# entn-at/tf-kaldi-speaker

Hardware: AMD Instinct MI355X
Metric: utterances/sec x-vector extraction (30-dim x 300-frame) (higher is better)
Workload: dtype f16+fp6-cross(f32-split); 1 GPU; tdnn x-vector (tdnn6_dense), statistics_pooling, 256 utt/GPU/step of 300 frames x 30 dims; batch_per_gpu=256, frames=300, node=tdnn6_dense, precision=f16f6, parallelism=utterance-shard x1, launch=stream launches

## Files before the change

### __graft_entry__.py

```python
import os
import subprocess
import sys

ROOT = os.path.dirname(os.path.abspath(__file__))
PKG = os.path.join(ROOT, "tf-kaldi-speaker_amd")
CSRC = os.path.join(PKG, "csrc")
LIB = os.path.join(PKG, "libxvec_hip.so")
SOURCES = ["gemm_f32.hip", "gemm_bf16x3.hip", "gemm_f6v2.hip", "gemm_f16f6.hip", "pool.hip", "grid.hip", "frontend.hip", "post.hip", "score.hip", "xvec_api.hip", "ark_io.cpp"]


AUDITED = ("gemm_bf16x3.hip", "gemm_f6v2.hip")


def audit_resources(remarks):
    import re
    kernels, cur = {}, None
    for line in remarks.splitlines():
        m = re.search(r"remark: Function Name: (\S+)", line)
        if m:
            cur = kernels.setdefault(m.group(1), {})
            continue
        m = re.search(r"remark:\s+([A-Za-z ]+?)(?: \[[^\]]*\])?: (\S+) \[-Rpass", line)
        if m and cur is not None:
            cur[m.group(1).strip()] = m.group(2)
    rows, bad = [], []
    for name, r in sorted(kernels.items()):
        if "w14p2" not in name and "w1p3" not in name and "gemm_f6v2_kernel" not in name:
            continue
        need_occ = 3
        rows.append("%s VGPRs %s SGPRs %s scratch %s vgpr_spill %s sgpr_spill %s occupancy %s"
                    % (name, r.get("VGPRs"), r.get("TotalSGPRs"), r.get("ScratchSize"), r.get("VGPRs Spill"),
                       r.get("SGPRs Spill"), r.get("Occupancy")))
        if r.get("ScratchSize") != "0" or r.get("VGPRs Spill") != "0" or int(r.get("Occupancy", "0")) < need_occ:
            bad.append(rows[-1])
    if len(rows) < 4:
        raise RuntimeError("resource audit: expected the hand-scheduled w14p2 / w1p3 kernels in the compiler remarks, found %d" % len(rows))
    os.makedirs(os.path.join(ROOT, "profiles", "r03"), exist_ok=True)
    with open(os.path.join(ROOT, "profiles", "r03", "gemm_resources.txt"), "w") as f:
        f.write("# hipcc -Rpass-analysis=kernel-resource-usage, csrc/gemm_bf16x3.hip + csrc/gemm_f6v2.hip (written by __graft_entry__.build)\n")
        f.write("\n".join(rows) + "\n")
    if bad:
        raise RuntimeError("resource audit failed (scratch / VGPR spill / too low an occupancy in a hand-counted-vmcnt kernel):\n"
                           + "\n".join(bad))
    print("[build] resource audit ok: %d hand-scheduled kernels, no scratch, no VGPR spill" % len(rows))


def audit_asm(asm_jobs):
    sys.path.insert(0, os.path.join(ROOT, "tools"))
    import asm_guard
    rows, bad = [], []
    for proc, cmd, asm in asm_jobs:
        if proc.wait() != 0:
            raise subprocess.CalledProcessError(proc.returncode, cmd)
        r, b = asm_guard.check_file(asm, want=("w14p2", "w1p3", "gemm_f6v2_kernel"), local=("w14p2", "w1p3"))
        rows += r
        bad += b
    if len(rows) < 4:
        raise RuntimeError("asm guard: expected the hand-scheduled kernels in the assembly, found %d" % len(rows))
    with open(os.path.join(ROOT, "profiles", "r03", "asm_guard.txt"), "w") as f:
        f.write("# tools/asm_guard.py on hipcc -S --cuda-device-only of csrc/gemm_bf16x3.hip + csrc/gemm_f6v2.hip (written by __graft_entry__.build)\n")
        f.write("\n".join(rows) + "\n")
    if bad:
        raise RuntimeError("asm guard failed:\n" + "\n".join(bad[:20]))
    print("[build] asm guard ok: %d kernels, no in-flight register touched, no compiler vector-memory instruction in a K loop" % len(rows))


def _stale():
    if not os.path.isfile(LIB):
        return True
    t = os.path.getmtime(LIB)
    deps = [os.path.join(CSRC, f) for f in os.listdir(CSRC)] + [os.path.join(ROOT, "include", "xvec_hip.h")]
    return any(os.path.getmtime(d) > t for d in deps)


def build(force=False):
    if force or _stale():
        objdir = os.path.join(PKG, "build")
        os.makedirs(objdir, exist_ok=True)
        flags = ["-O3", "-std=c++17", "--offload-arch=gfx950", "-fPIC", "-I", os.path.join(ROOT, "include")]
        flags += os.environ.get("XVEC_EXTRA_CFLAGS", "").split()
        jobs, asm_jobs = [], []
        for src in SOURCES:
            obj = os.path.join(objdir, os.path.splitext(src)[0] + ".o")
            cmd = ["hipcc"] + flags + ["-c", os.path.join(CSRC, src), "-o", obj]
            audit = src in AUDITED
            if audit:
                cmd.insert(1, "-Rpass-analysis=kernel-resource-usage")
# ... 61 lines not shown
```

### tf-kaldi-speaker_amd/csrc/gemm_bf16x3.hip

```cpp
#include <cstdlib>
#include <mutex>

#include "xv_f6.h"

namespace xv {

namespace {
constexpr int BM = 128, BN = 128;
constexpr int ROWB = 144;
constexpr int TILE_B = BM * ROWB;
typedef int i32x4 __attribute__((ext_vector_type(4)));
}

namespace {
constexpr int DROW = 128;
constexpr int DA_ROWS = 136;
constexpr int DA_BYTES = DA_ROWS * DROW;
constexpr int DB_BYTES = BN * DROW;
typedef __attribute__((address_space(1))) const void* gptr_t;
typedef __attribute__((address_space(3))) void* lptr_t;
}

#ifdef XV_LAB
__global__ __launch_bounds__(256, 2) void gemm_bf16x3_kernel(GemmArgs p, int nMt, int nNt) {
// ... 610 lines not shown
    mt = nMt + tile / nNt;
    nt = tile % nNt;
    const int per = cb_end / S;
    cb_begin = split * per;
    cb_end = cb_begin + per;
    p.Y = p.partial + ((int64_t)split * p.tail_mt - nMt) * (int64_t)BM * p.Npad;
    p.ldy = p.Npad;
    slice = true;
  } else if (EPI == 0 && (int)blockIdx.x >= nMt * nNt) {
    const int id = blockIdx.x - nMt * nNt;
    const int split = id % S, tile = id / S;
    mt = nMt + tile / nNt;
    nt = tile % nNt;
    const int per = cb_end / S;
    cb_begin = split * per;
    cb_end = cb_begin + per;
    p.Y = p.partial + ((int64_t)split * p.tail_mt - nMt) * (int64_t)BM * p.Npad;
    p.raw = 1;
    p.act = ACT_NONE;
    p.alpha = nullptr;
    p.ldy = p.Npad;
    p.N = p.Npad;
    p.M = (nMt + p.tail_mt) * BM;
    p.Ysb = nullptr;
    p.rowmap = nullptr;
    p.R = nullptr;
    p.pool_part = nullptr;
  } else {
    tile_of_block(blockIdx.x, nMt, nNt, mt, nt);
  }
  w14p2_tile<NPS, EPI, F16>(p, mt * BM, nt * BN, w, smem3, cb_begin, cb_end, slice);
}

__global__ void bf16x3_tail_reduce_kernel(GemmArgs p, int mt0, int S) {
  const int quads = p.Npad >> 2;
  const int64_t rows = (int64_t)p.tail_mt * BM;
  const int64_t total = rows * quads;
  for (int64_t i = (int64_t)blockIdx.x * blockDim.x + threadIdx.x; i < total; i += (int64_t)gridDim.x * blockDim.x) {
    const int64_t r = i / quads;
    const int n = (int)(i - r * quads) * 4;
    const int64_t m = (int64_t)mt0 * BM + r;
    if (m >= p.M) continue;
    bool zero;
    const int orow = out_row(p, (int)m, zero);
    if (orow < 0) continue;
    f32x4 acc = {0.f, 0.f, 0.f, 0.f};
    for (int s = 0; s < S; ++s) acc += *reinterpret_cast<const f32x4*>(p.partial + ((int64_t)s * rows + r) * p.Npad + n);
    f32x4 v = {0.f, 0.f, 0.f, 0.f};
#pragma unroll
    for (int e = 0; e < 4; ++e)
      if (n + e < p.N && !zero) v[e] = apply_act(fmaf(acc[e], p.scale[n + e], p.shift[n + e]), p.act, p.alpha ? p.alpha[n + e] : 0.f);
    if (p.Y && n < p.N) *reinterpret_cast<f32x4*>(p.Y + (int64_t)orow * p.ldy + n) = v;
    if (p.Ysb && n < p.ldsb) {
      uint32_t h01, l01, h23, l23;
      v *= p.sb_mul;
      split2(v[0], v[1], h01, l01, p.f16);
      split2(v[2], v[3], h23, l23, p.f16);
      if (p.f16) ovf_report(p.ovf, fmaxf(fmaxf(fabsf(v[0]), fabsf(v[1])), fmaxf(fabsf(v[2]), fabsf(v[3]))));
      char* blk = reinterpret_cast<char*>(p.Ysb) + (int64_t)orow * p.ldsb * 4 + (n >> 5) * 128 + (n & 31) * 2;
      *reinterpret_cast<uint2*>(blk) = make_uint2(h01, h23);
      *reinterpret_cast<uint2*>(blk + 64) = make_uint2(l01, l23);
    }
  }
}

#undef XV_GLD
// ... 154 lines not shown
    else       hipLaunchKernelGGL((gemm_bf16x3_w1p3_kernel<0, false, true>), grid, block, smemw1p3, s, a, nMain, nNt);
    return hipGetLastError();
  }
  if (a.ysb_f6 && (!a.f16 || (w > 1 && w < 5) || !a.Ysb || a.Y || a.R || a.pool_part)) return hipErrorInvalidValue;
  if (w == 1 && !tail && a.slab3) {
    if (a.ysb_f6) hipLaunchKernelGGL((gemm_bf16x3_w1p3_kernel<3, true>), grid, block, smemw1p3, s, a, nMain, nNt);
    else if (a.f16) hipLaunchKernelGGL((gemm_bf16x3_w1p3_kernel<0, true>), grid, block, smemw1p3, s, a, nMain, nNt);
    else       hipLaunchKernelGGL((gemm_bf16x3_w1p3_kernel<0, false>), grid, block, smemw1p3, s, a, nMain, nNt);
    return hipGetLastError();
  }
  const int S = tail ? a.ksplit : 0;
  const dim3 grid2(nMain * nNt + (tail ? a.tail_mt * nNt * a.ksplit : 0));
  if (a.ysb_f6) {
    if (w >= 5) hipLaunchKernelGGL((gemm_bf16x3_w14p2_kernel<1, 3, true>), grid2, block, smemw32, s, a, nMain, nNt, w, S);
    else        hipLaunchKernelGGL((gemm_bf16x3_w14p2_kernel<4, 3, true>), grid2, block, smemw32, s, a, nMain, nNt, w, S);
    const hipError_t e6 = hipGetLastError();
    if (e6 != hipSuccess || !tail) return e6;
    return launch_f6v2_tail_reduce(a, nMain, s);
  }
  if (w >= 5) {
    if (a.f16) hipLaunchKernelGGL((gemm_bf16x3_w14p2_kernel<1, 0, true>), grid2, block, smemw32, s, a, nMain, nNt, w, S);
    else       hipLaunchKernelGGL((gemm_bf16x3_w14p2_kernel<1, 0, false>), grid2, block, smemw32, s, a, nMain, nNt, w, S);
  } else {
    if (a.f16) hipLaunchKernelGGL((gemm_bf16x3_w14p2_kernel<4, 0, true>), grid2, block, smemw32, s, a, nMain, nNt, w, S);
    else       hipLaunchKernelGGL((gemm_bf16x3_w14p2_kernel<4, 0, false>), grid2, block, smemw32, s, a, nMain, nNt, w, S);
  }
  hipError_t e = hipGetLastError();
  if (e != hipSuccess || !tail) return e;
  const int64_t total = (int64_t)a.tail_mt * BM * (a.Npad >> 2);
  hipLaunchKernelGGL(bf16x3_tail_reduce_kernel, dim3((unsigned)((total + 255) / 256)), block, 0, s, a, nMain, a.ksplit);
  return hipGetLastError();
}

}

#ifdef XV_GEMM_TRACE
extern "C" int xvdbg_gemm_trace(long long* out, int max_wgs) {
  if (!xv::g_trace || xv::g_trace_wgs <= 0) return 0;
  const int n = xv::g_trace_wgs < max_wgs ? xv::g_trace_wgs : max_wgs;
  if (hipDeviceSynchronize() != hipSuccess) return -1;
  if (hipMemcpy(out, xv::g_trace, sizeof(long long) * 8 * n, hipMemcpyDeviceToHost) != hipSuccess) return -1;
  return n;
}
#endif
```

### tf-kaldi-speaker_amd/csrc/xv_kernels.h

```cpp
#pragma once
#include <hip/hip_runtime.h>
#include <stdint.h>

namespace xv {

enum Act : int { ACT_NONE = 0, ACT_RELU = 1, ACT_LRELU = 2, ACT_PRELU = 3, ACT_TANH = 4 };

constexpr float kLreluAlpha = 0.2f;
constexpr int kFlagWords = 8, kUttSmallWord = 4, kFeatMaxSlots = 32768;
constexpr float kVarFloor = 1e-12f;

struct GemmArgs {
  const float* X;
  int64_t ldx;
  int cin;
  int M;
  int K;
  int N;
  const float* Wt;
  int Kpad;
  int Npad;
  const float* scale;
  const float* shift;
  const float* alpha;
// ... 22 lines not shown
  int tail_mt = 0;
  float* pool_part;
  const int32_t* pool_row2utt;
  const int32_t* pool_slotbase;
  int64_t a_pitch;
  int64_t a_off;
  int64_t tap_stride;
  int ntaps;
  int ktap;
  const int32_t* arow;
  const float* R;
  int64_t ldr;
  const float* att_q = nullptr;
  float* att_part = nullptr;
  int64_t att_ld = 0;
  int att_heads = 0;
  const float* pool_w = nullptr;
  int pool_heads = 0;
  int pool_split = 0;
  int pool_dvh = 0;
  int pool_odim = 0;
};

hipError_t launch_gemm_f32(const GemmArgs& a, bool aligned, hipStream_t s);

int gemm_f32_ksplit(int M, int Kpad, int Npad);

int64_t gemm_bf16x3_tail_plan(int M, int Kpad, int Npad, int w, int* tail_mt, int* splits, int cb_quant = 1);

hipError_t launch_im2col_sb(const float* x, int64_t ldx, int cin, int w, int64_t rows, void* out_sb, int ldsb, int f16,
                            int* ovf, hipStream_t s);

hipError_t launch_gemm_bf16x3(const GemmArgs& a, hipStream_t s);
hipError_t launch_gemm_f16f6(const GemmArgs& a, hipStream_t s);
hipError_t launch_f6v2_tail_reduce(const GemmArgs& a, int nMain, hipStream_t s);
hipError_t launch_f6_from_sb(const void* sb, void* out, int64_t rows, int nblk, hipStream_t s);

hipError_t launch_build_rowmap(const int32_t* off0, int B, int ctx_in, int w, int32_t* rowmap, int M,
                               hipStream_t s);

hipError_t launch_stat_pool(const float* x, int64_t ldx, int C, const int32_t* off0, int B, int ctx,
                            float* out, int64_t ldo, hipStream_t s);

hipError_t launch_build_row2utt(const int32_t* off0, int B, int ctx, int32_t* row2utt, int M, hipStream_t s);
hipError_t launch_pool_finalize(const float* part, int C, const int32_t* off0, int B, int ctx,
                                const int32_t* slotbase, float* out, int64_t ldo, hipStream_t s);

hipError_t launch_build_rowmap_grid(const int32_t* off0, int B, int rows_per_t, int Fout, int So, int cover, int32_t* rowmap,
                                    int64_t M, hipStream_t s);
hipError_t launch_build_rowmap_grid_ts(const int32_t* off_in, const int32_t* off_out, int B, int rows_per_t, int Fout, int So,
                                       int ktime, int32_t* rowmap, int64_t M, hipStream_t s);
hipError_t launch_build_rowmap_grid_compact(const int32_t* off_in, const int32_t* off_out, int B, int Sin, int So, int Fout,
                                            int sw, int st, int ktime, int32_t* arow, int32_t* rowmap, int64_t M, int64_t Mpad,
                                            hipStream_t s);
hipError_t launch_grid_zero_border(const int32_t* off0, int B, int64_t frames, int F, int S, int chunks_y, int chunks_sb,
                                   float* y, void* ysb, hipStream_t s);
hipError_t launch_build_rowmap_rows(const int32_t* off0, int B, int32_t* rowmap, int64_t M, hipStream_t s);
hipError_t launch_build_rowmap_trows(const int32_t* off0, int B, int So, int32_t* rowmap, int64_t M, hipStream_t s);
hipError_t launch_build_rowmap_interior(const int32_t* off0, int B, int F, int S, int32_t* rowmap, int64_t M, hipStream_t s);
hipError_t launch_im2col2d_sb(const float* x, int64_t ldx, const int32_t* off0, int B, int F, int S, int64_t P, void* out_sb,
                              int f16, int* ovf, hipStream_t s);
hipError_t launch_im2col2d_f32(const float* x, int64_t ldx, const int32_t* off0, int B, int F, int S, int64_t P, float* out,
                               hipStream_t s);
hipError_t launch_conv0_direct(const float* x, int64_t ldx, const int32_t* off0, int B, int F, int S, int C, int64_t P,
                               const float* wdir, int act, const float* alpha, float* y, void* ysb, int ldsb, int f16, int* ovf,
                               float sb_mul, hipStream_t s);
// ... 67 lines not shown
```

### tf-kaldi-speaker_amd/csrc/xvec_api.hip

```cpp
#include <hip/hip_runtime.h>

#include <algorithm>
#include <cmath>
#include <cstdarg>
#include <cstdio>
#include <cstring>
#include <map>
#include <mutex>
#include <string>
#include <vector>

#include "../../include/xvec_hip.h"
#include "xv_kernels.h"

using namespace xv;

namespace {

constexpr double kBnEps = 1e-3;
constexpr int kSlackRows = 512;
constexpr int kAlign = 256;

thread_local std::string g_last_error;

// ... 86 lines not shown
  int sb_exp = 0;
};

struct Op {
  int kind = OP_GEMM;
  int layer = -1;
  int in0 = -1, in1 = -1;
  int out = -1;
  int bnvec = -1;
};

struct Node {
  std::string name;
  int op = -1;
  int stage = -1;
  bool att_weights = false;
};

}

struct xv_handle {
  xv_model_desc desc{};
  int device = 0;
  bool finalized = false;
  std::string err;
  std::mutex mu;
  std::mutex err_mu;
  std::mutex prof_mu;
  int opt_pool_fusion = 1;
  int opt_tail_split = 1;
  int opt_onetap_f6_notail = 1;
  int opt_grid_f6 = 1;
  int opt_slab3 = 1;
  int opt_grid_compact = 1;
  int opt_att_fusion = 1;
  int opt_profile_dominant = 0;
  std::mutex pool_mu;
  std::vector<DevBuf> pool;
  size_t pool_bytes = 0;
  std::map<std::string, HostTensor> tensors;
  std::vector<Layer> layers;
  std::vector<Value> values;
  std::vector<Op> ops;
  std::vector<Node> nodes;
  DevBuf query;
  DevBuf ovf_flag;
  DevBuf query_eff;
  int key_npad = 0;
  int att_dk_h = 0, att_dk = 0, att_dv = 0;
  int final_ctx = 14;
  std::string post_bn_scope, post_alpha_name;
  DevBuf post_vec;
  int pool_dim = 0;
  struct ProfRec { hipEvent_t e0, e1; const xv_plan* plan; int step; };
  bool profiling = false;
  std::vector<hipEvent_t> prof_pool;
  size_t prof_next = 0;
  std::vector<ProfRec> prof_recs;
  int prof_forwards = 0;
};

struct PlanStep {
  int op = -1;
  int stage = -1;
  bool to_out = false;
  int64_t out_off = -1;
  int64_t out_sb_off = -1;
  int64_t in0_off = -1, in1_off = -1;
  int64_t in0_sb_off = -1;
  int64_t rows_in = 0, rows_out = 0;
  int M = 0;
  int rowmap = -1;
  int64_t scratch_off = -1;
  int64_t scratch2_off = -1;
  int ksplit = 1;
  int tail_mt = 0;
  bool fuse_pool = false;
  int lvl_in = 0, lvl_out = 0;
  int64_t frames_out = 0;
  bool grid_cover = false;
  bool out_f6 = false;
  bool trows = false;
  bool in_f6 = false;
  bool compact = false;
  int arow = -1;
  int fuse_att = 0;
  int64_t att_w_off = -1;
  int64_t att_s0_off = -1;
  int64_t att_ld = 0;
  bool unpad_to_out = false;
  int64_t flops = 0, bytes = 0;
};

struct xv_plan {
  xv_handle* h = nullptr;
  xv_plan_info info{};
  std::vector<int32_t> offsets;
  std::vector<int32_t> offsets_slotbase;
  DevBuf d_offsets;
  std::vector<int32_t> lvl_offsets[4];
  DevBuf d_lvl[4];
  const int32_t* dev_offsets(int level) const {
    return static_cast<const int32_t*>(level > 0 ? d_lvl[level].p : d_offsets.p);
  }
  DevBuf d_rowmaps;
  std::vector<int64_t> rowmap_off;
  std::vector<PlanStep> steps;
  DevBuf d_row2utt;
  DevBuf d_slotbase;
  int64_t pool_slots = 0;
  bool uniform_len = true;
  int uniform_L = 0;
  int dominant_step = 0;
};

namespace {

int fail(xv_handle* h, int code, const char* fmt, ...) {
  char buf[512];
  va_list ap;
  va_start(ap, fmt);
  vsnprintf(buf, sizeof(buf), fmt, ap);
  va_end(ap);
  if (h) {
    std::lock_guard<std::mutex> lk(h->err_mu);
    h->err = buf;
  }
  g_last_error = buf;
  return code;
}

#define XV_HIP(h, expr)                                                                              \
  do {                                                                                               \
    hipError_t _e = (expr);                                                                          \
    if (_e != hipSuccess)                                                                            \
      return fail((h), XV_ERR_HIP, "%s failed: %s (%s:%d)", #expr, hipGetErrorString(_e), __FILE__,  \
                  __LINE__);                                                                         \
  } while (0)

int64_t align_up(int64_t v, int64_t a) { return (v + a - 1) / a * a; }

constexpr size_t kPoolMaxBuffers = 96, kPoolMaxBytes = (size_t)1 << 30;
// ... 732 lines not shown
        }
      XV_HIP(h, h->query_eff.alloc(qe.size() * sizeof(float)));
      XV_HIP(h, hipMemcpy(h->query_eff.p, qe.data(), qe.size() * sizeof(float), hipMemcpyHostToDevice));
    }
    if (h->desc.att_apply_nonlinear) {
      const int n = h->pool_dim;
      std::vector<double> s, t;
      bn_fold(h, h->post_bn_scope, n, s, t);
      std::vector<float> vec((size_t)3 * n, 0.f);
      for (int i = 0; i < n; ++i) { vec[i] = (float)s[i]; vec[(size_t)n + i] = (float)t[i]; }
      if (!h->post_alpha_name.empty()) {
        const auto& a = T(h, h->post_alpha_name).data;
        for (int i = 0; i < n; ++i) vec[(size_t)2 * n + i] = a[i];
      }
      XV_HIP(h, h->post_vec.alloc(vec.size() * sizeof(float)));
      XV_HIP(h, hipMemcpy(h->post_vec.p, vec.data(), vec.size() * sizeof(float), hipMemcpyHostToDevice));
    }
  }
  XV_HIP(h, h->ovf_flag.alloc((kFlagWords + kFeatMaxSlots) * sizeof(int)));
  XV_HIP(h, hipMemset(h->ovf_flag.p, 0, (kFlagWords + kFeatMaxSlots) * sizeof(int)));
  XV_HIP(h, hipDeviceSynchronize());
  for (auto& kv : h->tensors) { kv.second.data.clear(); kv.second.data.shrink_to_fit(); }
  h->finalized = true;
  return XV_OK;
}

int xv_set_option(xv_handle* h, const char* name, int value) {
  if (!h || !name) return fail(h, XV_ERR_INVALID, "xv_set_option: null argument");
  std::lock_guard<std::mutex> lk(h->mu);
  if (!strcmp(name, "pool_fusion")) h->opt_pool_fusion = value != 0;
  else if (!strcmp(name, "tail_split")) h->opt_tail_split = value != 0;
  else if (!strcmp(name, "att_fusion")) h->opt_att_fusion = value != 0;
  else if (!strcmp(name, "slab3")) h->opt_slab3 = value != 0;
  else if (!strcmp(name, "onetap_f6_notail")) h->opt_onetap_f6_notail = value != 0;
  else if (!strcmp(name, "grid_f6")) h->opt_grid_f6 = value != 0;
  else if (!strcmp(name, "grid_compact")) h->opt_grid_compact = value != 0;
  else if (!strcmp(name, "profile_dominant")) h->opt_profile_dominant = value != 0;
  else return fail(h, XV_ERR_INVALID, "xv_set_option: unknown option '%s'", name);
  return XV_OK;
}

int xv_check_overflow(xv_handle* h, int reset) {
  if (!h) return fail(nullptr, XV_ERR_INVALID, "xv_check_overflow: null handle");
  if (!h->finalized || !h->ovf_flag.p) return 0;
  DeviceGuard g(h->device);
  std::vector<int32_t> w((size_t)kFlagWords + kFeatMaxSlots);
  XV_HIP(h, hipMemcpy(w.data(), h->ovf_flag.p, w.size() * sizeof(int32_t), hipMemcpyDeviceToHost));
  int32_t v[2] = {w[0], w[1]};
  for (int i = 0; i < kFeatMaxSlots; ++i) v[1] = std::max(v[1], w[(size_t)kFlagWords + i]);
  if (w[kUttSmallWord]) v[1] = w[kUttSmallWord];
  if (reset) XV_HIP(h, hipMemset(h->ovf_flag.p, 0, w.size() * sizeof(int32_t)));
  return xv_flags_decode(v);
}

int xv_flags_decode(const int32_t* flags) {
  if (!flags) return XV_ERR_INVALID;
  if (flags[0]) return 1;
  if (flags[1] > 0) {
    float mx;
    memcpy(&mx, &flags[1], 4);
    if (mx < 0.00390625f) return 2;
  }
  return 0;
}

int xv_flags_async(xv_handle* h, int32_t* host_flags, void* stream) {
// ... 222 lines not shown
      if (L.mode == 0) st.M = (int)(st.rows_in - (L.w - 1));
      else if (L.mode == 1 && L.use_f6) {
        st.trows = true;
        st.M = (int)padded_rows;
      }
      else if ((L.mode == 1 || L.mode == 2) && L.use_split && h->opt_grid_compact &&
               st.rows_in * (int64_t)sb_ld(L.cin) * 4 < ((int64_t)1 << 32)) {
        st.compact = true;
        st.M = (int)(Fl[st.lvl_out] * L.Fout);
      }
      else if (L.mode == 1 || L.mode == 2) st.M = (int)(padded_rows * (h->values[op.in0].grid_S / L.sw));
      else if (L.mode == 3) st.M = (int)padded_rows;
      else st.M = (int)(padded_rows * h->values[op.out].grid_S);
      if (st.compact || st.trows) st.grid_cover = false;
      else if (L.mode == 1 || L.mode == 2) st.grid_cover = L.st == 1 && h->values[op.in0].grid_S / L.sw == h->values[op.out].grid_S;
      else if (L.mode == 4) st.grid_cover = true;
      if (L.w > 1 || L.mode != 0) {
        st.rowmap = (int)p->rowmap_off.size();
        p->rowmap_off.push_back(rowmap_elems);
        rowmap_elems += align_up(st.M, 64);
        if (st.compact) {
          st.arow = (int)p->rowmap_off.size();
          p->rowmap_off.push_back(rowmap_elems);
          rowmap_elems += align_up(st.M, 128);
        }
      }
      const int64_t valid_out = L.mode == 0 ? st.rows_out : Fl[st.lvl_out] * (L.mode == 3 ? 1 : L.Fout);
      st.flops = 2 * valid_out * (int64_t)L.cout * L.K();
      st.bytes = 4 * (st.rows_in * L.cin + st.rows_out * L.cout + (int64_t)L.K() * L.cout);
      int64_t scratch = 0;
      if (L.mode == 4) {
        scratch = ((int64_t)st.M + kSlackRows) * 32 * 4;
      } else if (L.im2col) {
        scratch = L.cin_pad ? (st.rows_in + kSlackRows) * (int64_t)L.cin_pad * 4 : (st.M + kSlackRows) * (int64_t)L.Kpad * 4;
      } else if (!L.use_split && op.out != fused_value) {
        st.ksplit = gemm_f32_ksplit(st.M, L.Kpad, L.Npad);
        if (st.ksplit > 1) scratch = (int64_t)st.ksplit * st.M * L.Npad * 4;
      } else if (L.use_f6) {
        scratch = (st.rows_in + kSlackRows) * (int64_t)sb_ld(L.cin) * 4;
        if (h->opt_tail_split && op.in1 <= 0 && L.mode == 0) {
          const int64_t part = gemm_bf16x3_tail_plan(st.M, L.Kpad, L.Npad, L.w, &st.tail_mt, &st.ksplit, 4);
          if (part > 0) {
            step_scratch2 = align_up(part, kAlign);
            st.scratch2_off = arena_alloc(step_scratch2);
          }
        }
      } else if (L.use_split && L.mode == 0 && op.out != fused_value && op.in1 <= 0 && h->opt_tail_split &&
                 order[s] != key_prod && order[s] != val_prod) {
        scratch = gemm_bf16x3_tail_plan(st.M, L.Kpad, L.Npad, L.w, &st.tail_mt, &st.ksplit);
      }
      if (scratch > 0) {
        step_scratch = align_up(scratch, kAlign);
        st.scratch_off = arena_alloc(step_scratch);
      }
    } else if (op.kind == OP_AFFINE_ACT) {
      st.stage = st.to_out ? node.stage : 2;
      st.bytes = 8 * st.rows_out * h->values[op.out].cols;
    } else if (op.kind == OP_ATT_POOL && val_prod >= 0) {
      st.fuse_att = 1;
      st.bytes = 4 * (p->pool_slots * (2 * (h->pool_dim / 2) + h->desc.att_num_heads) + st.rows_out * h->values[op.out].cols);
      st.flops = 8 * p->pool_slots * (h->pool_dim / 2);
    } else if (op.kind == OP_STAT_POOL || op.kind == OP_ATT_POOL) {
      st.bytes = 4 * (st.rows_in * h->values[op.in0].cols + st.rows_out * h->values[op.out].cols);
      st.flops = 4 * st.rows_in * h->values[op.in0].cols;
      if (op.kind == OP_STAT_POOL && op.in0 == fused_value) {
        st.fuse_pool = true;
// ... 169 lines not shown
      const Layer& L = h->layers[op.layer];
      const int ctx_in = h->values[op.in0].ctx;
      const int32_t* doff = p->dev_offsets(st.lvl_in);
      int32_t* rm = static_cast<int32_t*>(p->d_rowmaps.p) + p->rowmap_off[st.rowmap];
      if (L.mode == 0) e = launch_build_rowmap(doff, batch, ctx_in, L.w, rm, st.M, s);
      else if (st.trows) e = launch_build_rowmap_trows(doff, batch, h->values[op.out].grid_S, rm, st.M, s);
      else if (st.compact)
        e = launch_build_rowmap_grid_compact(doff, p->dev_offsets(st.lvl_out), batch, h->values[op.in0].grid_S,
                                             h->values[op.out].grid_S, L.Fout, L.sw, L.st, L.mode == 1 ? 3 : 1,
                                             static_cast<int32_t*>(p->d_rowmaps.p) + p->rowmap_off[st.arow], rm, st.M,
                                             align_up(st.M, 128), s);
      else if ((L.mode == 1 || L.mode == 2) && L.st == 2)
        e = launch_build_rowmap_grid_ts(doff, p->dev_offsets(st.lvl_out), batch, h->values[op.in0].grid_S / L.sw, L.Fout,
                                        h->values[op.out].grid_S, L.mode == 1 ? 3 : 1, rm, st.M, s);
      else if (L.mode == 1 || L.mode == 2)
        e = launch_build_rowmap_grid(doff, batch, h->values[op.in0].grid_S / L.sw, L.Fout, h->values[op.out].grid_S,
                                     st.grid_cover ? 1 : 0, rm, st.M, s);
      else if (L.mode == 3) e = launch_build_rowmap_rows(doff, batch, rm, st.M, s);
      else e = launch_build_rowmap_interior(doff, batch, L.Fout, h->values[op.out].grid_S, rm, st.M, s);
      if (e != hipSuccess) return bail(e, "build_rowmap");
    }
  }
  if (slot_value >= 0) {
    const int ctx = h->values[slot_value].ctx;
    const int64_t rows = value_rows(h, slot_value, Fl, batch);
    if ((e = pool_take(h, (size_t)rows * 4, p->d_row2utt)) != hipSuccess) return bail(e, "hipMalloc(row2utt)");
    if ((e = pool_take(h, (size_t)batch * 4, p->d_slotbase)) != hipSuccess) return bail(e, "hipMalloc(slotbase)");
    if ((e = hipMemcpyAsync(p->d_slotbase.p, p->offsets_slotbase.data(), (size_t)batch * 4, hipMemcpyHostToDevice, s)) != hipSuccess)
      return bail(e, "hipMemcpyAsync(slotbase)");
    if ((e = launch_build_row2utt(p->dev_offsets(h->values[slot_value].tlevel), batch, ctx,
                                  static_cast<int32_t*>(p->d_row2utt.p), (int)rows, s)) != hipSuccess)
      return bail(e, "build_row2utt");
  }
  *out = p;
  return XV_OK;
}

int xv_plan_query(const xv_plan* p, xv_plan_info* info) {
  if (!p || !info) return XV_ERR_INVALID;
  *info = p->info;
  return XV_OK;
}

void xv_plan_destroy(xv_plan* p) {
  if (!p) return;
  {
    DeviceGuard g(p->h->device);
    pool_give(p->h, p->d_offsets);
    for (int k = 1; k < 4; ++k) pool_give(p->h, p->d_lvl[k]);
    pool_give(p->h, p->d_rowmaps);
    pool_give(p->h, p->d_row2utt);
    pool_give(p->h, p->d_slotbase);
  }
  delete p;
}

static const char* step_name(const xv_handle* h, const PlanStep& st) {
  const Op& op = h->ops[st.op];
  switch (op.kind) {
    case OP_GEMM: {
      const Layer& L = h->layers[op.layer];
      if (!L.ep[ST_AFFINE].empty()) return L.ep[ST_AFFINE].c_str();
      const size_t a = L.kernel_name.find('/'), b = L.kernel_name.rfind('/');
      static thread_local std::string tmp;
      tmp = (a != std::string::npos && b > a) ? L.kernel_name.substr(a + 1, b - a - 1) : L.kernel_name;
      return tmp.c_str();
    }
    case OP_STAT_POOL: return "stat_pool";
    case OP_ATT_SCORES: return "att_scores";
    case OP_ATT_SOFTMAX: return "att_softmax";
    case OP_ATT_POOL: return "att_pool";
    case OP_AFFINE_ACT: return "att_post";
    case OP_L2_SCALE: return "l2_scale";
    case OP_GRID_MAXPOOL: return "conv0_max";
    default: return "op";
  }
}

static int run_plan(xv_handle* h, const xv_plan* p, const float* feats, int feat_ld, float* out, int64_t out_cap,
                    void* workspace, int64_t ws_bytes, hipStream_t s) {
  if (!h || !p) return fail(h, XV_ERR_INVALID, "xv_forward: null handle/plan");
  if (p->h != h) return fail(h, XV_ERR_INVALID, "xv_forward: plan belongs to another handle");
  if (!feats || !out) return fail(h, XV_ERR_INVALID, "xv_forward: null feature/output pointer");
  if (feat_ld < h->desc.feat_dim) return fail(h, XV_ERR_INVALID, "xv_forward: feat_ld %d < feature_dim %d", feat_ld, h->desc.feat_dim);
  if (out_cap < p->info.out_rows * p->info.out_cols)
// ... 113 lines not shown
        if (st.out_sb_off >= 0) {
          a.Ysb = ws + st.out_sb_off;
          a.ldsb = sb_ld(L.cout);
          if (st.out_off < 0 && !st.to_out) a.Y = nullptr;
        }
        if (L.mode == 4) {
          if (st.scratch_off < 0) return fail(h, XV_ERR_STATE, "conv0 has no scratch");
          a.cin = 32; a.K = 32;
          const bool direct = L.use_split && !st.to_out && st.stage == L.final_stage() && L.cout % 8 == 0 &&
                              (st.out_sb_off < 0 || L.cout % 32 == 0) && L.cout <= 256 && L.wdir.p;
          if (direct) {
            XV_HIP(h, launch_conv0_direct(feats, feat_ld, off, B, L.Fout, vo.grid_S, L.cout, st.M, static_cast<const float*>(L.wdir.p),
                                          L.act, L.d_alpha(), st.out_off >= 0 ? reinterpret_cast<float*>(ws + st.out_off) : nullptr,
                                          st.out_sb_off >= 0 ? ws + st.out_sb_off : nullptr, sb_ld(L.cout), f16,
                                          static_cast<int*>(h->ovf_flag.p), a.sb_mul, s));
            break;
          }
          if (L.use_split) {
            XV_HIP(h, launch_im2col2d_sb(feats, feat_ld, off, B, L.Fout, vo.grid_S, st.M, ws + st.scratch_off, f16, static_cast<int*>(h->ovf_flag.p), s));
            a.Xsb = ws + st.scratch_off; a.ldsbx = 32; a.Wsb = L.wsb.p; a.Wfr = L.wfr.p;
            XV_HIP(h, launch_gemm_bf16x3(a, s));
          } else {
            XV_HIP(h, launch_im2col2d_f32(feats, feat_ld, off, B, L.Fout, vo.grid_S, st.M, reinterpret_cast<float*>(ws + st.scratch_off), s));
            a.X = reinterpret_cast<const float*>(ws + st.scratch_off); a.ldx = 32;
            XV_HIP(h, launch_gemm_f32(a, true, s));
          }
          if (st.unpad_to_out)
            XV_HIP(h, launch_grid_unpad_n(reinterpret_cast<const float*>(ws + st.out_off), off_out, B, vo.grid_F, vo.grid_S, vo.cols,
                                          st.frames_out, out, s));
          break;
        }
        if (L.im2col) {
          if (st.scratch_off < 0) return fail(h, XV_ERR_STATE, "im2col layer has no scratch");
          if (L.cin_pad) {
            XV_HIP(h, launch_im2col_sb(feats, feat_ld, L.cin, 1, st.rows_in, ws + st.scratch_off, L.cin_pad, f16,
                                       static_cast<int*>(h->ovf_flag.p), s));
            if (f16) XV_HIP(h, launch_feat_utt_guard(feats, feat_ld, L.cin, off, B, static_cast<int*>(h->ovf_flag.p), s));
            a.Xsb = ws + st.scratch_off;
            a.ldsbx = L.cin_pad;
            a.cin = L.cin_pad;
            a.K = L.w * L.cin_pad;
            a.Wsb = L.wsb.p; a.Wfr = L.wfr.p;
            a.ysb_f6 = st.out_f6 ? 1 : 0;
            XV_HIP(h, launch_gemm_bf16x3(a, s));
            break;
          }
          XV_HIP(h, launch_im2col_sb(feats, feat_ld, L.cin, L.w, st.M, ws + st.scratch_off, L.Kpad, f16, static_cast<int*>(h->ovf_flag.p), s));
          if (f16) XV_HIP(h, launch_feat_utt_guard(feats, feat_ld, L.cin, off, B, static_cast<int*>(h->ovf_flag.p), s));
          a.Xsb = ws + st.scratch_off;
          a.ldsbx = L.Kpad;
          a.cin = a.K;
          a.Wsb = L.wsb.p; a.Wfr = L.wfr.p;
          XV_HIP(h, launch_gemm_bf16x3(a, s));
          break;
        }
        if (L.use_f6) {
          if (st.in0_sb_off < 0 || st.scratch_off < 0) return fail(h, XV_ERR_STATE, "f16f6 layer %s has no input / scratch", L.kernel_name.c_str());
          if (st.in_f6) {
            a.Xsb = ws + st.in0_sb_off;
          } else {
            XV_HIP(h, launch_f6_from_sb(ws + st.in0_sb_off, ws + st.scratch_off, st.rows_in, sb_ld(L.cin) / 32, s));
            a.Xsb = ws + st.scratch_off;
          }
          a.ysb_f6 = st.out_f6 ? 1 : 0;
          if (!st.in_f6)
            XV_HIP(h, hipMemsetAsync(const_cast<char*>(static_cast<const char*>(a.Xsb)) + st.rows_in * (int64_t)sb_ld(L.cin) * 4, 0,
// ... 423 lines not shown
```

Baseline: 226,700 utterances/s.

## Add streaming first-layer GEMM fusing im2col, split and overflow guard

```diff
diff --git a/__graft_entry__.py b/__graft_entry__.py
--- a/__graft_entry__.py
+++ b/__graft_entry__.py
@@ -25,9 +25,9 @@
             cur[m.group(1).strip()] = m.group(2)
     rows, bad = [], []
     for name, r in sorted(kernels.items()):
-        if "w14p2" not in name and "w1p3" not in name and "gemm_f6v2_kernel" not in name:
+        if "w14p2" not in name and "w1p3" not in name and "gemm_f6v2_kernel" not in name and "l1s_kernel" not in name:
             continue
-        need_occ = 3
+        need_occ = 2 if "l1s_kernel" in name else 3
         rows.append("%s VGPRs %s SGPRs %s scratch %s vgpr_spill %s sgpr_spill %s occupancy %s"
                     % (name, r.get("VGPRs"), r.get("TotalSGPRs"), r.get("ScratchSize"), r.get("VGPRs Spill"),
                        r.get("SGPRs Spill"), r.get("Occupancy")))
@@ -52,7 +52,7 @@
     for proc, cmd, asm in asm_jobs:
         if proc.wait() != 0:
             raise subprocess.CalledProcessError(proc.returncode, cmd)
-        r, b = asm_guard.check_file(asm, want=("w14p2", "w1p3", "gemm_f6v2_kernel"), local=("w14p2", "w1p3"))
+        r, b = asm_guard.check_file(asm, want=("w14p2", "w1p3", "gemm_f6v2_kernel", "l1s_kernel"), local=("w14p2", "w1p3", "l1s_kernel"))
         rows += r
         bad += b
     if len(rows) < 4:
diff --git a/tf-kaldi-speaker_amd/csrc/gemm_bf16x3.hip b/tf-kaldi-speaker_amd/csrc/gemm_bf16x3.hip
--- a/tf-kaldi-speaker_amd/csrc/gemm_bf16x3.hip
+++ b/tf-kaldi-speaker_amd/csrc/gemm_bf16x3.hip
@@ -666,6 +666,177 @@
   w14p2_tile<NPS, EPI, F16>(p, mt * BM, nt * BN, w, smem3, cb_begin, cb_end, slice);
 }
 
+#define XV_WAIT8(N, a, b, c, d, e, f, g, h)                                                                                  \
+  asm volatile("s_waitcnt vmcnt(%8)" : "+v"(a), "+v"(b), "+v"(c), "+v"(d), "+v"(e), "+v"(f), "+v"(g), "+v"(h) : "n"(N))
+template <int EPI, bool F16>
+__global__ __launch_bounds__(256, 2) void gemm_bf16x3_l1s_kernel(GemmArgs p, int nMt, int nNt, int w, const int32_t* __restrict__ tile_first,
+                                                                 const int32_t* __restrict__ utt_off) {
+  extern __shared__ __attribute__((aligned(16))) char smem3[];
+  char* As = smem3;
+  char* scratch = smem3 + DA_BYTES;
+  const int tid = threadIdx.x;
+  const int lane = tid & 63;
+  const int wave = __builtin_amdgcn_readfirstlane(tid >> 6);
+  const int c16 = lane & 15, g4 = lane >> 4;
+  const int mt = xcd_remap(blockIdx.x, nMt);
+  const int m0 = mt * BM;
+  const int R = BM + w - 1;
+  const int64_t rows_in = (int64_t)p.M + w - 1;
+  const int cin = p.cin;
+
+  const int64_t nkb4k = (int64_t)(p.Kpad >> 5) * 4096;
+  const char* Wg = reinterpret_cast<const char*>(p.Wfr) + (int64_t)wave * nkb4k + lane * 16;
+  bf16x8 W0[4], W1[4], W2[4];
+  {
+    const char* q1 = Wg + 4096;
+    XV_GLD(W0[0], Wg, 0); XV_GLD(W0[1], Wg, 1024); XV_GLD(W0[2], Wg, 2048); XV_GLD(W0[3], Wg, 3072);
+    XV_GLD(W1[0], q1, 0); XV_GLD(W1[1], q1, 1024); XV_GLD(W1[2], q1, 2048); XV_GLD(W1[3], q1, 3072);
+  }
+
+  float* rowmax = reinterpret_cast<float*>(scratch);
+  int* pend = reinterpret_cast<int*>(scratch + 1024);
+  float* wred = reinterpret_cast<float*>(scratch + 1040);
+  {
+    float va[9], vb[9];
+#pragma unroll
+    for (int it = 0; it < 9; ++it) {
+      const int i = it * 256 + tid, r = i >> 4, k = (i & 15) * 2;
+      const int64_t m = (int64_t)m0 + r;
+      const bool ok = r < R && m < rows_in;
+      va[it] = (ok && k < cin) ? p.X[m * p.ldx + k] : 0.f;
+      vb[it] = (ok && k + 1 < cin) ? p.X[m * p.ldx + k + 1] : 0.f;
+    }
+    float mx = 0.f;
+    bool bad = false;
+#pragma unroll
+    for (int it = 0; it < 9; ++it) {
+      const int i = it * 256 + tid, r = i >> 4, pr = i & 15;
+      uint32_t hi, lo;
+      split2t<F16>(va[it], vb[it], hi, lo);
+      if (r < DA_ROWS) {
+        const int sw = ((r >> 1) & 3) << 1;
+        char* row = As + r * DROW + (pr & 3) * 4;
+        *reinterpret_cast<uint32_t*>(row + (((pr >> 2) ^ sw) << 4)) = hi;
+        *reinterpret_cast<uint32_t*>(row + (((4 + (pr >> 2)) ^ sw) << 4)) = lo;
+      }
+      if constexpr (F16) {
+        float pm = fmaxf(fabsf(va[it]), fabsf(vb[it]));
+        bad |= !(pm <= kF16Max);
+        mx = fmaxf(mx, pm);
+#pragma unroll
+        for (int o = 8; o > 0; o >>= 1) pm = fmaxf(pm, __shfl_xor(pm, o, 64));
+        if (pr == 0) rowmax[r] = pm;
+      }
+    }
+    if constexpr (F16) {
+      if (p.ovf) {
+        if (bad) *p.ovf = 1;
+#pragma unroll
+        for (int o = 32; o > 0; o >>= 1) mx = fmaxf(mx, __shfl_xor(mx, o, 64));
+        if (lane == 0) reinterpret_cast<float*>(p.ovf + kFlagWords)[blockIdx.x * 4 + wave] = (mx <= 3.0e38f) ? mx : 0.f;
+      }
+      if (tid == 0) pend[0] = -1;
+    }
+  }
+  asm volatile("s_waitcnt vmcnt(0)" ::: "memory");
+  __syncthreads();
+
+  if constexpr (F16) {
+    if (p.ovf && tile_first) {
+      const int f0 = tile_first[mt], f1 = tile_first[mt + 1];
+      for (int u = f0 + tid; u < f1; u += 256) {
+        const int b = utt_off[u], e = utt_off[u + 1];
+        const int r1 = min(e - m0, R);
+        float um = 0.f;
+        for (int r = b - m0; r < r1; ++r) um = fmaxf(um, rowmax[r]);
+        if (e - m0 > R && um < 0.00390625f) {
+          pend[0] = e;
+          pend[1] = __float_as_int(um);
+        } else if (um > 0.f && um < 0.00390625f) {
+          p.ovf[kUttSmallWord] = __float_as_int(um);
+        }
+      }
+      __syncthreads();
+      const int e = pend[0];
+      if (e >= 0) {
+        const int64_t rb = (int64_t)m0 + R, n = ((int64_t)e - rb) * cin;
+        float um = 0.f;
+        for (int64_t i = tid; i < n; i += 256) {
+          const int64_t r = i / cin;
+          um = fmaxf(um, fabsf(p.X[(rb + r) * p.ldx + (i - r * cin)]));
+        }
+#pragma unroll
+        for (int o = 32; o > 0; o >>= 1) um = fmaxf(um, __shfl_xor(um, o, 64));
+        if (lane == 0) wred[wave] = um;
+        __syncthreads();
+        if (tid == 0) {
+          um = fmaxf(fmaxf(fmaxf(wred[0], wred[1]), fmaxf(wred[2], wred[3])), __int_as_float(pend[1]));
+          if (um > 0.f && um < 0.00390625f) p.ovf[kUttSmallWord] = __float_as_int(um);
+        }
+      }
+      __syncthreads();
+    }
+  }
+
+  for (int nt = 0; nt < nNt; ++nt) {
+    const char* Wt = Wg + (int64_t)nt * 4 * nkb4k;
+    if (nt > 0) {
+      XV_GLD(W0[0], Wt, 0); XV_GLD(W0[1], Wt, 1024); XV_GLD(W0[2], Wt, 2048); XV_GLD(W0[3], Wt, 3072);
+      const char* Wt1 = Wt + 4096;
+      XV_GLD(W1[0], Wt1, 0); XV_GLD(W1[1], Wt1, 1024); XV_GLD(W1[2], Wt1, 2048); XV_GLD(W1[3], Wt1, 3072);
+      XV_WAIT8(0, W0[0], W0[1], W0[2], W0[3], W1[0], W1[1], W1[2], W1[3]);
+    }
+    f32x4 acc[8][2];
+#pragma unroll
+    for (int i = 0; i < 8; ++i)
+#pragma unroll
+      for (int c = 0; c < 2; ++c) acc[i][c] = f32x4{0.f, 0.f, 0.f, 0.f};
+    auto step = [&](int j, bf16x8 (&Wc)[4], bf16x8 (&Wn)[4]) __attribute__((always_inline)) {
+      const char* q = Wt + (int64_t)(j + 2 < w ? j + 2 : 0) * 4096;
+      const char* ab = As + (c16 + j) * DROW;
+      const int aswz = (((c16 + j) >> 1) & 3) << 1;
+      const int off_hi = (g4 ^ aswz) << 4, off_lo = ((4 + g4) ^ aswz) << 4;
+      bf16x8 fh[8], fl[8];
+      auto read_frag = [&](int ft) {
+        fh[ft] = *reinterpret_cast<const bf16x8*>(ab + off_hi + ft * (16 * DROW));
+        fl[ft] = *reinterpret_cast<const bf16x8*>(ab + off_lo + ft * (16 * DROW));
+      };
+      read_frag(0);
+      read_frag(1);
+      __builtin_amdgcn_sched_barrier(0);
+#pragma unroll
+      for (int g = 0; g < 8; ++g) {
+        if (g == 0) XV_GLD(Wn[0], q, 0);
+        if (g == 2) XV_GLD(Wn[1], q, 1024);
+        if (g == 4) XV_GLD(Wn[2], q, 2048);
+        if (g == 6) XV_GLD(Wn[3], q, 3072);
+        if (g + 2 < 8) read_frag(g + 2);
+        if (g == 0) XV_WAIT4(5, Wc[0], Wc[1], Wc[2], Wc[3]);
+        acc[g][0] = mfma_split16<F16>(Wc[0], fl[g], acc[g][0]);
+        acc[g][1] = mfma_split16<F16>(Wc[1], fl[g], acc[g][1]);
+        acc[g][0] = mfma_split16<F16>(Wc[2], fh[g], acc[g][0]);
+        acc[g][1] = mfma_split16<F16>(Wc[3], fh[g], acc[g][1]);
+        acc[g][0] = mfma_split16<F16>(Wc[0], fh[g], acc[g][0]);
+        acc[g][1] = mfma_split16<F16>(Wc[1], fh[g], acc[g][1]);
+        __builtin_amdgcn_sched_barrier(0);
+      }
+    };
+    for (int j = 0; j < w; j += 3) {
+      step(j, W0, W2);
+      if (j + 1 < w) step(j + 1, W1, W0);
+      if (j + 2 < w) step(j + 2, W2, W1);
+    }
+    XV_WAIT8(0, W0[0], W0[1], W0[2], W0[3], W1[0], W1[1], W1[2], W1[3]);
+    XV_WAIT4(0, W2[0], W2[1], W2[2], W2[3]);
+    __builtin_amdgcn_sched_barrier(0);
+    int lane_e = lane;
+    asm volatile("" : "+v"(lane_e));
+    if constexpr (EPI == 3) store_wave_tile_n32_f6(p, acc, m0, nt * BN + wave * 32, lane_e, wave, scratch);
+    else store_wave_tile_n32<64, F16>(p, acc, m0, nt * BN + wave * 32, lane_e, wave, scratch);
+  }
+}
+#undef XV_WAIT8
+
 __global__ void bf16x3_tail_reduce_kernel(GemmArgs p, int mt0, int S) {
   const int quads = p.Npad >> 2;
   const int64_t rows = (int64_t)p.tail_mt * BM;
@@ -886,6 +1057,42 @@
   return hipGetLastError();
 }
 
+bool gemm_l1_stream_ok(int M, int cin, int w, int Npad) {
+  return M > 0 && cin >= 1 && cin <= 32 && w >= 2 && w <= 9 && Npad % BN == 0 && (M + BM - 1) / BM <= kFeatMaxSlots / 4;
+}
+
+hipError_t launch_gemm_l1_stream(const GemmArgs& a, int w, const int32_t* tile_first, const int32_t* utt_off, hipStream_t s) {
+  if (a.M <= 0) return hipSuccess;
+  if (!gemm_l1_stream_ok(a.M, a.cin, w, a.Npad) || a.Kpad != w * 32 || !a.X || !a.Wfr || a.R || a.pool_part || a.att_part || a.pool_w ||
+      a.a_pitch || a.arow || a.raw || (a.N & 3))
+    return hipErrorInvalidValue;
+  if (a.ysb_f6 && (!a.f16 || w < 5 || !a.Ysb || a.Y)) return hipErrorInvalidValue;
+  static std::mutex init_mu;
+  static bool attr_set[64] = {};
+  const size_t smem = (size_t)DA_BYTES + 4 * 8192;
+  int dev = 0;
+  if (hipGetDevice(&dev) != hipSuccess) dev = 0;
+  {
+    std::lock_guard<std::mutex> init_lock(init_mu);
+    if (!attr_set[dev & 63]) {
+      const void* kernels[] = {reinterpret_cast<const void*>(gemm_bf16x3_l1s_kernel<0, false>),
+                               reinterpret_cast<const void*>(gemm_bf16x3_l1s_kernel<0, true>),
+                               reinterpret_cast<const void*>(gemm_bf16x3_l1s_kernel<3, true>)};
+      for (const void* k : kernels) {
+        const hipError_t r = hipFuncSetAttribute(k, hipFuncAttributeMaxDynamicSharedMemorySize, (int)smem);
+        if (r != hipSuccess) return r;
+      }
+      attr_set[dev & 63] = true;
+    }
+  }
+  const int nNt = a.Npad / BN, nMt = (a.M + BM - 1) / BM;
+  const dim3 grid(nMt), block(256);
+  if (a.ysb_f6) hipLaunchKernelGGL((gemm_bf16x3_l1s_kernel<3, true>), grid, block, smem, s, a, nMt, nNt, w, tile_first, utt_off);
+  else if (a.f16) hipLaunchKernelGGL((gemm_bf16x3_l1s_kernel<0, true>), grid, block, smem, s, a, nMt, nNt, w, tile_first, utt_off);
+  else hipLaunchKernelGGL((gemm_bf16x3_l1s_kernel<0, false>), grid, block, smem, s, a, nMt, nNt, w, tile_first, utt_off);
+  return hipGetLastError();
+}
+
 }
 
 #ifdef XV_GEMM_TRACE
diff --git a/tf-kaldi-speaker_amd/csrc/xv_kernels.h b/tf-kaldi-speaker_amd/csrc/xv_kernels.h
--- a/tf-kaldi-speaker_amd/csrc/xv_kernels.h
+++ b/tf-kaldi-speaker_amd/csrc/xv_kernels.h
@@ -78,6 +78,8 @@
                             int* ovf, hipStream_t s);
 
 hipError_t launch_gemm_bf16x3(const GemmArgs& a, hipStream_t s);
+bool gemm_l1_stream_ok(int M, int cin, int w, int Npad);
+hipError_t launch_gemm_l1_stream(const GemmArgs& a, int w, const int32_t* tile_first, const int32_t* utt_off, hipStream_t s);
 hipError_t launch_gemm_f16f6(const GemmArgs& a, hipStream_t s);
 hipError_t launch_f6v2_tail_reduce(const GemmArgs& a, int nMain, hipStream_t s);
 hipError_t launch_f6_from_sb(const void* sb, void* out, int64_t rows, int nblk, hipStream_t s);
diff --git a/tf-kaldi-speaker_amd/csrc/xvec_api.hip b/tf-kaldi-speaker_amd/csrc/xvec_api.hip
--- a/tf-kaldi-speaker_amd/csrc/xvec_api.hip
+++ b/tf-kaldi-speaker_amd/csrc/xvec_api.hip
@@ -142,6 +142,7 @@
   int opt_onetap_f6_notail = 1;
   int opt_grid_f6 = 1;
   int opt_slab3 = 1;
+  int opt_l1_stream = 1;
   int opt_grid_compact = 1;
   int opt_att_fusion = 1;
   int opt_profile_dominant = 0;
@@ -192,6 +193,7 @@
   bool out_f6 = false;
   bool trows = false;
   bool in_f6 = false;
+  bool l1_stream = false;
   bool compact = false;
   int arow = -1;
   int fuse_att = 0;
@@ -218,6 +220,8 @@
   std::vector<PlanStep> steps;
   DevBuf d_row2utt;
   DevBuf d_slotbase;
+  std::vector<int32_t> l1_first;
+  DevBuf d_l1_first;
   int64_t pool_slots = 0;
   bool uniform_len = true;
   int uniform_L = 0;
@@ -1016,6 +1020,7 @@
   else if (!strcmp(name, "tail_split")) h->opt_tail_split = value != 0;
   else if (!strcmp(name, "att_fusion")) h->opt_att_fusion = value != 0;
   else if (!strcmp(name, "slab3")) h->opt_slab3 = value != 0;
+  else if (!strcmp(name, "l1_stream")) h->opt_l1_stream = value != 0;
   else if (!strcmp(name, "onetap_f6_notail")) h->opt_onetap_f6_notail = value != 0;
   else if (!strcmp(name, "grid_f6")) h->opt_grid_f6 = value != 0;
   else if (!strcmp(name, "grid_compact")) h->opt_grid_compact = value != 0;
@@ -1304,6 +1309,16 @@
       if (L.mode == 4) {
         scratch = ((int64_t)st.M + kSlackRows) * 32 * 4;
       } else if (L.im2col) {
+        st.l1_stream = h->opt_l1_stream && L.cin_pad == 32 && L.mode == 0 && L.wfr.p && (L.cout & 3) == 0 && st.rowmap >= 0 &&
+                       L.Kpad == L.w * 32 && gemm_l1_stream_ok(st.M, L.cin, L.w, L.Npad);
+        if (st.l1_stream) {
+          const int nMt = (st.M + 127) / 128;
+          p->l1_first.assign((size_t)nMt + 1, batch);
+          for (int t = 0, u = 0; t < nMt; ++t) {
+            while (u < batch && p->offsets[u] < (int64_t)t * 128) ++u;
+            p->l1_first[t] = u;
+          }
+        }
         scratch = L.cin_pad ? (st.rows_in + kSlackRows) * (int64_t)L.cin_pad * 4 : (st.M + kSlackRows) * (int64_t)L.Kpad * 4;
       } else if (!L.use_split && op.out != fused_value) {
         st.ksplit = gemm_f32_ksplit(st.M, L.Kpad, L.Npad);
@@ -1539,6 +1554,11 @@
                                   static_cast<int32_t*>(p->d_row2utt.p), (int)rows, s)) != hipSuccess)
       return bail(e, "build_row2utt");
   }
+  if (!p->l1_first.empty()) {
+    if ((e = pool_take(h, p->l1_first.size() * 4, p->d_l1_first)) != hipSuccess) return bail(e, "hipMalloc(l1_first)");
+    if ((e = hipMemcpyAsync(p->d_l1_first.p, p->l1_first.data(), p->l1_first.size() * 4, hipMemcpyHostToDevice, s)) != hipSuccess)
+      return bail(e, "hipMemcpyAsync(l1_first)");
+  }
   *out = p;
   return XV_OK;
 }
@@ -1558,6 +1578,7 @@
     pool_give(p->h, p->d_rowmaps);
     pool_give(p->h, p->d_row2utt);
     pool_give(p->h, p->d_slotbase);
+    pool_give(p->h, p->d_l1_first);
   }
   delete p;
 }
@@ -1737,6 +1758,12 @@
         }
         if (L.im2col) {
           if (st.scratch_off < 0) return fail(h, XV_ERR_STATE, "im2col layer has no scratch");
+          if (st.l1_stream) {
+            a.Wfr = L.wfr.p;
+            a.ysb_f6 = st.out_f6 ? 1 : 0;
+            XV_HIP(h, launch_gemm_l1_stream(a, L.w, f16 ? static_cast<const int32_t*>(p->d_l1_first.p) : nullptr, off, s));
+            break;
+          }
           if (L.cin_pad) {
             XV_HIP(h, launch_im2col_sb(feats, feat_ld, L.cin, 1, st.rows_in, ws + st.scratch_off, L.cin_pad, f16,
                                        static_cast<int*>(h->ovf_flag.p), s));
```

New measurement: 219,600 utterances/s. 3.1% lower.
